# HongwenZhang/DaNet-DensePose2SMPL

Measured on NVIDIA H100. Metric: images/sec DaNet fwd bs=64 224x224 (HRNet-W48 + part regressors + SMPL LBS + IUV render), higher is better.
Workload: dtype split-f16 operands (hi+lo, 22 bits; 3 MMAs per K step), f32 accumulate

## Files before the change

### danet-densepose2smpl_b200/_lib.py

```python
import ctypes
import os

_HERE = os.path.dirname(os.path.abspath(__file__))
LIB_PATH = os.path.join(_HERE, "libdanet_b200.so")

c_int, c_i64, c_f, c_p = ctypes.c_int32, ctypes.c_int64, ctypes.c_float, ctypes.c_void_p


class SmplDesc(ctypes.Structure):
    _fields_ = [("num_verts", c_int), ("num_joints", c_int), ("num_betas", c_int),
                ("v_template", c_p), ("shapedirs", c_p), ("posedirs", c_p), ("J_regressor", c_p),
                ("lbs_weights", c_p), ("parents", c_p),
                ("num_selected", c_int), ("selected_verts", c_p),
                ("num_extra", c_int), ("J_regressor_extra", c_p),
                ("num_h36m", c_int), ("J_regressor_h36m", c_p),
                ("num_out_joints", c_int), ("joint_map", c_p)]


class RasterDesc(ctypes.Structure):
    _fields_ = [("num_smpl_verts", c_int), ("num_mesh_verts", c_int), ("vert_mapping", c_p),
                ("num_faces", c_int), ("faces", c_p), ("textures", c_p),
                ("orig_size", c_int), ("out_size", c_int), ("focal_length", c_f),
                ("near_plane", c_f), ("far_plane", c_f), ("tex_mode", c_int)]

# ... 30 lines not shown
SIGNATURES = {
    "danet_last_error": (ctypes.c_char_p, []),
    "danet_version": (c_int, []),
    "danet_device_info": (c_int, [c_p, c_p, c_p]),
    "danet_smpl_create": (c_int, [ctypes.POINTER(SmplDesc), ctypes.POINTER(c_p)]),
    "danet_smpl_destroy": (c_int, [c_p]),
    "danet_smpl_workspace_bytes": (c_i64, [c_p, c_int]),
    "danet_smpl_forward": (c_int, [c_p, c_int, c_p, c_p, c_int, c_p, c_p, c_p, c_p, c_p, c_p, c_int, c_p]),
    "danet_smpl_backward_workspace_bytes": (c_i64, [c_p, c_int]),
    "danet_smpl_backward": (c_int, [c_p, c_int, c_p, c_p, c_p, c_p, c_p, c_p, c_p, c_p]),
    "danet_rot6d_to_rotmat": (c_int, [c_int, c_p, c_p, c_p]),
    "danet_batch_rodrigues": (c_int, [c_int, c_p, c_p, c_int, c_p]),
    "danet_perspective_projection": (c_int, [c_int, c_int, c_p, c_p, c_p, c_p, c_p, c_p, c_p]),
    "danet_mpjpe_h36m": (c_int, [c_int, c_p, c_p, c_p, c_p]),
    "danet_body_uv_losses_workspace_bytes": (c_i64, [c_int, c_int]),
    "danet_body_uv_losses": (c_int, [c_int, c_int, c_int, c_int, c_i64, c_i64, c_p, c_p, c_p, c_p, c_p, c_p, c_p, c_p,
                                     c_p, c_f, c_f, c_p, c_p, c_p, c_p, c_p, c_p, c_p]),
    "danet_dp_uvia_losses_workspace_bytes": (c_i64, [c_int, c_int]),
    "danet_dp_uvia_losses": (c_int, [c_int, c_int, c_int, c_int] + [c_p] * 12 + [c_int, c_f, c_f, c_f] + [c_p] * 7),
    "danet_stn_kps_losses_workspace_bytes": (c_i64, [c_int, c_int]),
    "danet_stn_kps_losses": (c_int, [c_int, c_int, c_int, c_p, c_p, c_int, c_f, c_f, c_p, c_p, c_p, c_p, c_p]),
    "danet_part_iuv_targets": (c_int, [c_int, c_int, c_int, c_p, c_p, c_p, c_p, c_int, c_p, c_p]),
    "danet_raster_create": (c_int, [ctypes.POINTER(RasterDesc), ctypes.POINTER(c_p)]),
    "danet_raster_destroy": (c_int, [c_p]),
    "danet_raster_workspace_bytes": (c_i64, [c_p, c_int]),
    "danet_raster_iuv": (c_int, [c_p, c_int, c_p, c_p, c_p, c_p, c_p, c_p, c_p, c_p, c_p, c_p]),
    "danet_iuv_img2map": (c_int, [c_int, c_int, c_p, c_p, c_p, c_p, c_p, c_p]),
    "danet_conv_tc_packed_bytes": (c_i64, [ctypes.POINTER(ConvDesc)]),
    "danet_conv_tc_pack": (c_int, [ctypes.POINTER(ConvDesc), c_p, c_p, c_p]),
    "danet_conv_tc_supported": (c_int, [ctypes.POINTER(ConvDesc)]),
    "danet_conv_tc_geometry": (c_int, [ctypes.POINTER(ConvDesc), c_p]),
    "danet_conv_tc_cta_geometry": (c_int, [ctypes.POINTER(ConvDesc), c_p]),
    "danet_conv_tc_dispatch": (c_int, [ctypes.POINTER(ConvDesc), c_p]),
    "danet_conv_tc_group": (c_int, [c_int, ctypes.POINTER(ConvProblem), c_p]),
    "danet_conv_tc_config": (c_int, [c_int, ctypes.POINTER(ConvDesc), c_p]),
    "danet_conv_weights_simt": (c_int, [c_int] * 6 + [c_p, c_p, c_p]),
    "danet_conv_dgrad_pieces": (c_int, [c_int, c_int, c_p]),
    "danet_conv_dgrad_weights": (c_int, [c_int] * 5 + [c_p, c_int, c_int, c_p, c_p, c_p]),
    "danet_conv_dgrad_scatter": (c_int, [c_int] * 9 + [c_p, ctypes.POINTER(c_p), c_p, c_p, c_int, c_p, c_p]),
    "danet_conv_grad_split": (c_int, [c_int] * 4 + [c_p] * 5),
    "danet_conv_wgrad_workspace_bytes": (c_i64, [ctypes.POINTER(ConvDesc)]),
    "danet_conv_wgrad": (c_int, [ctypes.POINTER(ConvDesc), c_int, c_int, ctypes.POINTER(Act), ctypes.POINTER(Act), c_p, c_p,
                                 c_p, c_p, c_p]),
    "danet_conv_bias_grad_workspace_bytes": (c_i64, [c_int, c_int, c_int]),
    "danet_conv_bias_grad": (c_int, [c_int, c_int, c_int, c_p, c_p, c_p, c_p]),
    "danet_bn2d_workspace_bytes": (c_i64, [c_int, c_int, c_int]),
    "danet_bn2d_forward": (c_int, [c_int, c_int, c_int] + [c_p] * 5 + [c_int, c_f, c_f, c_p, c_int] + [c_p] * 5),
    "danet_bn2d_backward": (c_int, [c_int, c_int, c_int] + [c_p] * 5 + [c_int, c_int] + [c_p] * 6),
    "danet_maxpool3x3s2_nchw_forward": (c_int, [c_int] * 4 + [c_p] * 4),
    "danet_maxpool3x3s2_nchw_backward": (c_int, [c_int] * 4 + [c_p] * 4),
    "danet_global_avgpool_backward": (c_int, [c_int, c_int, c_p, c_p, c_p]),
    "danet_linear_backward": (c_int, [c_int] * 3 + [c_p] * 7),
    "danet_hr_fuse_forward": (c_int, [c_int] * 5 + [c_p, c_p, c_int, c_p, c_p]),
    "danet_hr_fuse_backward": (c_int, [c_int] * 5 + [c_p] * 4),
    "danet_part_crops_forward": (c_int, [c_int] * 3 + [c_p, c_p, c_int, c_p, c_p]),
    "danet_part_crops_backward": (c_int, [c_int] * 3 + [c_p, c_p, c_int, c_p, c_p]),
    "danet_part_thetas": (c_int, [c_int] * 3 + [c_p] * 4 + [c_f, c_p, c_f, c_p, c_f, c_int, c_p, c_p, c_p]),
    "danet_act_split": (c_int, [c_i64, c_p, c_p, c_p, c_p]),
    "danet_act_merge": (c_int, [c_i64, c_p, c_p, c_p, c_p]),
    "danet_global_avgpool": (c_int, [c_int, c_int, c_int, ctypes.POINTER(Act), c_p, c_p]),
    "danet_linear": (c_int, [c_int, c_int, c_int, c_p, c_p, c_p, c_p, c_p, c_p]),
    "danet_iuvmap_clean_nchw": (c_int, [c_int, c_int, c_int, c_int, c_p, c_p, c_p, c_p, c_p, c_p, c_p, c_p, c_p]),
    "danet_gcn_head_train_workspace_bytes": (c_i64, [c_int]),
    "danet_gcn_head_train_forward": (c_int, [c_int, ctypes.POINTER(GcnTrainParams), c_int] + [c_p] * 9),
    "danet_gcn_head_train_backward": (c_int, [c_int, ctypes.POINTER(GcnTrainParams), c_int] + [c_p] * 9),
    "danet_gcn_head_losses": (c_int, [c_int] + [c_p] * 6 + [c_f, c_f] + [c_p] * 5),
# ... 62 lines not shown
```

### danet-densepose2smpl_b200/csrc/conv_tc.cu

```cuda
#include "common.cuh"
#include "wgmma_f16.cuh"
#include "tc_ptx.cuh"
#include <cuda.h>
#include <cuda_fp16.h>
#include <mutex>
#include <utility>
#include <string.h>
#include <math.h>

namespace danet {
namespace tc {

constexpr int kTileH = 16, kTileW = 8;
constexpr int kConsFast = 2, kThreadsFast = (4 * kConsFast + 1) * 32;
constexpr int kWarpProd = 4 * kConsFast;
constexpr int kConsExact = 4, kThreadsExact = 4 * kConsExact * 32;
constexpr int kNtMaxExact = 64, kNtMaxFast = 256;
constexpr int kMaxAStages = 8, kMaxBStages = 8;
constexpr int kSmemMax = 227 * 1024;
constexpr int kSmemFixed = 2048;
constexpr int kSchedDepth = 4, kSchedAhead = 2, kSchedStatic = 3;
constexpr int kPackHeader = 1024;
constexpr int kSegMmas = 8;
__host__ __device__ constexpr bool seg_close(bool last_block, int seg_mmas) { return last_block || seg_mmas >= kSegMmas; }

struct alignas(64) Prob {
    CUtensorMap tm[2];
    const uint8_t* wpk; const float* bias;
    const float* res_f; const __half* res_hi; const __half* res_lo;
    float* y_f; __half* y_hi; __half* y_lo;
    int N, H, W, Cin, Cout, Ho, Wo, ks, stride, pad, relu, wsets, exact;
    int npa;
    int SWB, KCH, nchunks;
    int TG;
    int NT, ntn;
    int nstack, hs, box_h;
    int bpc;
    int par_py[4], par_px[4], ntap[4], ngrp[4], stage_bytes, sbo_a;
    int tapoff16[4][16];
    int tapidx[4][16];
    int tiles_w, tiles_h, tile_count;
    int rows_blk;
    int tap_bytes, b_block_bytes, nblk;
    long long blocks_per_set;
    unsigned long long m_ntn, m_tw, m_th, m_ws;
};

constexpr int kMaxProb = 6;
struct ArgsN {
    int nprob, total_units, na_stages, a_slot_bytes, nb_stages, b_slot_bytes;
    unsigned* sched;
    Prob p[kMaxProb];
    int unit_base[kMaxProb], unit_count[kMaxProb];
};

static unsigned long long magic40(int d) { return (1ull << 40) / (unsigned long long)d + 1ull; }

static bool make_prob(const danet_conv_desc* d, Prob* g) {
    if (!(d->stride == 1 || d->stride == 2) || !(d->ksize == 1 || d->ksize == 3 || d->ksize == 7) || d->pad != d->ksize / 2) return false;
    if (d->Cin % 8 != 0 || d->Cout % 8 != 0 || d->H < 1 || d->W < 1 || d->N < 1 || d->wsets < 1) return false;
    g->N = d->N; g->H = d->H; g->W = d->W; g->Cin = d->Cin; g->Cout = d->Cout; g->ks = d->ksize;
    g->pad = d->pad; g->stride = d->stride; g->relu = d->relu; g->wsets = d->wsets;
    g->exact = (d->flags & DANET_CONV_EXACT) ? 1 : 0;
    g->Ho = (d->H + 2 * d->pad - d->ksize) / d->stride + 1;
    g->Wo = (d->W + 2 * d->pad - d->ksize) / d->stride + 1;
    if (g->Ho < 1 || g->Wo < 1) return false;
    const int np = (d->Cout + 15) / 16 * 16;
    const int ntmax = g->exact ? kNtMaxExact : kNtMaxFast;
    g->ntn = (np + ntmax - 1) / ntmax;
    g->NT = ((np + g->ntn - 1) / g->ntn + 15) / 16 * 16;
    g->npa = 0;
    int max_ntap = 0, tr_max = 0, tc_max = 0;
    int tc_[4];
    for (int py = 0; py < d->stride; ++py)
        for (int px = 0; px < d->stride; ++px) {
            const int tr = py < d->ksize ? (d->ksize - 1 - py) / d->stride + 1 : 0;
            const int tcn = px < d->ksize ? (d->ksize - 1 - px) / d->stride + 1 : 0;
            if (tr * tcn == 0) continue;
            if (tr * tcn > 16) return false;
            const int a = g->npa++;
            g->par_py[a] = py; g->par_px[a] = px; g->ntap[a] = tr * tcn; tc_[a] = tcn;
            max_ntap = tr * tcn > max_ntap ? tr * tcn : max_ntap;
            tr_max = tr > tr_max ? tr : tr_max; tc_max = tcn > tc_max ? tcn : tc_max;
        }
    const int Hb = kTileH + tr_max - 1, Wb = kTileW + tc_max - 1;
    g->nstack = 1; g->hs = kTileH; g->box_h = Hb;
    if (d->stride == 1 && d->H + d->pad <= kTileH / 2) {
        g->hs = d->H + d->pad;
        g->box_h = d->H + 2 * d->pad;
    } else if (d->stride == 2 && g->Ho + tr_max - 1 <= kTileH / 2) {
        g->hs = g->box_h = g->Ho + tr_max - 1;
    }
    int swb = 128;
    const int c16 = (d->Cin + 15) / 16 * 16;
    while (swb > 32 && swb / 2 >= 2 * c16) swb /= 2;
    if (g->hs < kTileH && (g->hs * Wb * swb) % 128 != 0) { g->hs = kTileH; g->box_h = Hb; }
    if (g->hs < kTileH) g->nstack = kTileH / g->hs;
    g->SWB = swb; g->KCH = swb / 2;
    g->nchunks = (d->Cin + g->KCH - 1) / g->KCH;
    g->rows_blk = g->NT * (g->exact ? 2 : 1);
    g->tap_bytes = g->rows_blk * swb;
    int tg = max_ntap;
    while (tg > 1 && tg * g->tap_bytes > (g->exact ? 24 : 48) * 1024) --tg;
    g->TG = tg;
    g->b_block_bytes = (tg * g->tap_bytes + 1023) / 1024 * 1024;
    g->stage_bytes = Hb * Wb * swb; g->sbo_a = Wb * swb;
    g->bpc = 0;
    for (int a = 0; a < 4; ++a) {
        if (a >= g->npa) { g->par_py[a] = g->par_px[a] = g->ntap[a] = g->ngrp[a] = 0;
                           for (int k = 0; k < 16; ++k) g->tapoff16[a][k] = g->tapidx[a][k] = 0; continue; }
        g->ngrp[a] = (g->ntap[a] + tg - 1) / tg;
        g->bpc += g->ngrp[a];
        for (int k = 0; k < 16; ++k) { g->tapoff16[a][k] = 0; g->tapidx[a][k] = 0; }
        for (int k = 0; k < g->ntap[a]; ++k) {
            const int ti = k / tc_[a], tj = k % tc_[a];
            g->tapoff16[a][k] = ((ti * Wb + tj) * swb) >> 4;
            g->tapidx[a][k] = (g->par_py[a] + d->stride * ti) * d->ksize + (g->par_px[a] + d->stride * tj);
        }
    }
    g->nblk = g->nchunks * g->bpc;
    g->blocks_per_set = (long long)g->ntn * g->nblk;
    g->tiles_w = (g->Wo + kTileW - 1) / kTileW; g->tiles_h = (g->Ho + kTileH - 1) / kTileH;
    const long long groups = g->nstack == 1 ? d->N
                           : (long long)d->wsets * (((d->N + d->wsets - 1) / d->wsets + g->nstack - 1) / g->nstack);
    const long long tiles = groups * g->tiles_h * g->tiles_w * g->ntn;
    if (tiles >= (1 << 24) || g->wsets >= (1 << 16)) return false;
    if ((long long)d->N * g->Ho * g->Wo * d->Cout >= (1LL << 31) || (long long)d->N * d->H * d->W * d->Cin >= (1LL << 31)) return false;
    g->tile_count = (int)tiles;
    g->m_ntn = magic40(g->ntn); g->m_tw = magic40(g->tiles_w); g->m_th = magic40(g->tiles_h); g->m_ws = magic40(g->wsets);
    return true;
}

static int pair_count(const Prob& g) {
    const int U = g.tiles_h * g.tiles_w * g.ntn;
    const int groups = g.tile_count / U;
    if (g.tiles_h > 1) return groups * ((g.tiles_h + 1) / 2) * g.tiles_w * g.ntn;
    const int per_set = (groups + g.wsets - 1) / g.wsets;
    return (per_set + 1) / 2 * g.wsets * U;
}

static bool plan_rings(ArgsN* a) {
    int amax = 0, bmax = 0, need_a = 2, max_a = kMaxAStages;
    bool exact = false;
    for (int i = 0; i < a->nprob; ++i) {
        amax = a->p[i].stage_bytes > amax ? a->p[i].stage_bytes : amax;
        bmax = a->p[i].b_block_bytes > bmax ? a->p[i].b_block_bytes : bmax;
        if (a->p[i].exact) exact = true;
    }
    a->a_slot_bytes = (amax + 1023) / 1024 * 1024;
    a->b_slot_bytes = (bmax + 1023) / 1024 * 1024;
    if (exact) {
        a->a_slot_bytes *= 2;
        need_a = max_a = 3;
    }
    int nb = 3;
    int na = (kSmemMax - kSmemFixed - nb * a->b_slot_bytes) / a->a_slot_bytes;
    if (na < need_a) { nb = 2; na = (kSmemMax - kSmemFixed - nb * a->b_slot_bytes) / a->a_slot_bytes; }
    if (na < need_a) return false;
    if (na > max_a) na = max_a;
    while (nb < kMaxBStages && kSmemFixed + na * a->a_slot_bytes + (nb + 1) * a->b_slot_bytes <= kSmemMax) ++nb;
    a->na_stages = na; a->nb_stages = nb;
    return true;
}

__device__ __forceinline__ uint64_t make_desc(uint32_t saddr, uint32_t sbo_bytes, uint32_t swb) {
    const uint32_t mode = swb == 128 ? 1u : (swb == 64 ? 2u : 3u);
    const uint32_t lo = ((saddr >> 4) & 0x3FFFu) | (1u << 16);
    const uint32_t hi = ((sbo_bytes >> 4) & 0x3FFFu) | (mode << 30);
    return ((uint64_t)hi << 32) | lo;
}
__host__ __device__ __forceinline__ uint32_t swz(uint32_t off, uint32_t mask) { return off ^ (((off >> 7) & mask) << 4); }
__host__ __device__ __forceinline__ int mdiv(int x, unsigned long long m) { return (int)(((unsigned long long)(unsigned)x * m) >> 40); }

struct TileCoord { int nt, tw, th, img0, ws; };
__host__ __device__ __forceinline__ void group_coord(const Prob& g, int grp, TileCoord& c) {
    const int bg = mdiv(grp, g.m_ws);
    c.ws = grp - bg * g.wsets;
    c.img0 = c.ws + g.wsets * bg * g.nstack;
}
__device__ __forceinline__ TileCoord decode_tile(const Prob& g, int t) {
    TileCoord c;
    int r = mdiv(t, g.m_ntn); c.nt = t - r * g.ntn;
    int r2 = mdiv(r, g.m_tw); c.tw = r - r2 * g.tiles_w;
    const int grp = mdiv(r2, g.m_th); c.th = r2 - grp * g.tiles_h;
    group_coord(g, grp, c);
    return c;
}

__host__ __device__ __forceinline__ TileCoord pair_coord(const Prob& g, int pp, int h) {
    TileCoord c;
    const int r = mdiv(pp, g.m_ntn); c.nt = pp - r * g.ntn;
    const int outer = mdiv(r, g.m_tw); c.tw = r - outer * g.tiles_w;
    int grp;
    if (g.tiles_h > 1) {
        const int th2 = (g.tiles_h + 1) >> 1;
        grp = outer / th2;
        c.th = 2 * (outer - grp * th2) + h;
    } else {
        const int q = mdiv(outer, g.m_ws);
        grp = (2 * q + h) * g.wsets + (outer - q * g.wsets);
        c.th = 0;
    }
    group_coord(g, grp, c);
    return c;
}

struct Ring { int as, bs; uint32_t aph, bph; };

struct Smem { uint32_t sA, sB, bar_a_full, bar_a_empty, bar_b_full, bar_b_empty; };

constexpr uint32_t kOffSchedFull = 512, kOffSchedEmpty = kOffSchedFull + 8 * kSchedDepth;
constexpr uint32_t kOffSchedRing = kOffSchedFull + 16 * kSchedDepth, kOffCursor = 640, kOffPark = 768;

enum CursorField {
    kCurSeq, kCurPub, kCurPubEnd,
    kCurPi,
    kCurC, kCurSlot, kCurStep,
    kCurH0, kCurH1, kCurW0,
    kCurImg0, kCurImg1, kCurBlk,
    kCurFa, kCurFb,
    kCurRa, kCurRb,
    kCurAs, kCurBs, kCurAph, kCurBph,
    kCurFields
};
static_assert(kOffCursor + 4 * kCurFields <= kOffPark && kOffPark + 4 * 32 <= 1024, "barrier region layout");

__device__ __forceinline__ int sched_next(const Smem& S, int seq) {
// ... 19 lines not shown
    asm volatile("ld.shared.s32 %0, [%1];" : "=r"(v) : "r"(cur + 4 * f) : "memory");
    return v;
}
__device__ __forceinline__ void cur_set(uint32_t cur, int f, int v) {
    asm volatile("st.shared.s32 [%0], %1;" ::"r"(cur + 4 * f), "r"(v) : "memory");
}

__device__ __forceinline__ void produce(const ArgsN& a, const Smem& S, int dA, int dB) {
    const uint32_t cur = S.bar_a_full + kOffCursor;
    cur_set(cur, kCurRa, cur_get(cur, kCurRa) + dA);
    cur_set(cur, kCurRb, cur_get(cur, kCurRb) + dB);
#pragma unroll 1
    for (;;) {
        if (cur_get(cur, kCurPi) < 0) {
#pragma unroll 1
            while (cur_get(cur, kCurPub) <= cur_get(cur, kCurSeq) + kSchedAhead && !cur_get(cur, kCurPubEnd)) {
                const int pub = cur_get(cur, kCurPub), rs = pub & (kSchedDepth - 1);
                mbar_wait_inl(S.bar_a_full + kOffSchedEmpty + 8 * rs, ((pub / kSchedDepth) & 1) ^ 1);
                const int t = sched_unit(a, pub, [&] { return __shfl_sync(0xffffffffu, atom_inc_elect(a.sched), 0); });
                if (t == a.total_units) cur_set(cur, kCurPubEnd, 1);
                st_arrive_elect(S.bar_a_full + kOffSchedRing + 4 * rs, t, S.bar_a_full + kOffSchedFull + 8 * rs);
                cur_set(cur, kCurPub, pub + 1);
            }
            int pair;
            asm volatile("ld.shared.s32 %0, [%1];" : "=r"(pair)
                         : "r"(S.bar_a_full + kOffSchedRing + 4 * (cur_get(cur, kCurSeq) & (kSchedDepth - 1))) : "memory");
            pair = __shfl_sync(0xffffffffu, pair, 0);
            if (pair >= a.total_units) return;
            const int pi = unit_prob(a, pair);
            const Prob& P = a.p[pi];
            const int pp = pair - a.unit_base[pi];
            {
                const TileCoord tc = pair_coord(P, pp, 0);
                cur_set(cur, kCurH0, tc.th * kTileH * P.stride - P.pad);
                cur_set(cur, kCurW0, tc.tw * kTileW * P.stride - P.pad);
                cur_set(cur, kCurImg0, tc.img0);
                cur_set(cur, kCurBlk, tc.ws * (int)P.blocks_per_set + tc.nt * P.nblk);
            }
            {
                const TileCoord tc = pair_coord(P, pp, 1);
                cur_set(cur, kCurH1, tc.th * kTileH * P.stride - P.pad);
                cur_set(cur, kCurImg1, tc.img0);
            }
            cur_set(cur, kCurC, 0); cur_set(cur, kCurSlot, 0); cur_set(cur, kCurStep, 0);
            cur_set(cur, kCurPi, pi);
        }
        const Prob& P = a.p[cur_get(cur, kCurPi)];
        const int step = cur_get(cur, kCurStep);
        if (step < 2) {
            if (cur_get(cur, kCurFa) >= cur_get(cur, kCurRa) + a.na_stages) return;
            {
                const int as = cur_get(cur, kCurAs);
                mbar_wait_inl(S.bar_a_empty + 8 * as, ((cur_get(cur, kCurAph) >> as) & 1) ^ 1);
                mbar_expect_tx_elect(S.bar_a_full + 8 * as, 2u * P.nstack * P.box_h * P.sbo_a);
            }
#pragma unroll 1
            for (int k = 0; k < 2 * P.nstack; ++k) {
                const int h = k >= P.nstack ? 1 : 0, n = k - h * P.nstack, slot = cur_get(cur, kCurSlot), as = cur_get(cur, kCurAs);
                tma_load_4d_elect(S.sA + as * a.a_slot_bytes + h * (a.a_slot_bytes >> 1) + n * P.hs * P.sbo_a,
                                  &P.tm[step], cur_get(cur, kCurC) * P.KCH, cur_get(cur, kCurW0) + P.par_px[slot],
                                  cur_get(cur, kCurH0 + h) + P.par_py[slot], cur_get(cur, kCurImg0 + h) + n * P.wsets,
                                  S.bar_a_full + 8 * as);
            }
            const int as = cur_get(cur, kCurAs);
            cur_set(cur, kCurAph, cur_get(cur, kCurAph) ^ (1 << as));
            cur_set(cur, kCurAs, as + 1 == a.na_stages ? 0 : as + 1);
            cur_set(cur, kCurFa, cur_get(cur, kCurFa) + 1);
            cur_set(cur, kCurStep, step + 1);
        } else {
            if (cur_get(cur, kCurFb) >= cur_get(cur, kCurRb) + a.nb_stages) return;
            {
                const int bs = cur_get(cur, kCurBs);
                mbar_wait_inl(S.bar_b_empty + 8 * bs, ((cur_get(cur, kCurBph) >> bs) & 1) ^ 1);
                const uint32_t bar = S.bar_b_full + 8 * bs;
                mbar_expect_tx_elect(bar, (uint32_t)P.b_block_bytes);
                bulk_g2s_elect(S.sB + bs * a.b_slot_bytes, P.wpk + kPackHeader + (long long)cur_get(cur, kCurBlk) * P.b_block_bytes,
                               (uint32_t)P.b_block_bytes, bar);
                cur_set(cur, kCurBph, cur_get(cur, kCurBph) ^ (1 << bs));
                cur_set(cur, kCurBs, bs + 1 == a.nb_stages ? 0 : bs + 1);
            }
            cur_set(cur, kCurFb, cur_get(cur, kCurFb) + 1);
            cur_set(cur, kCurBlk, cur_get(cur, kCurBlk) + 1);
            const int slot = cur_get(cur, kCurSlot);
            if (step - 1 < P.ngrp[slot]) cur_set(cur, kCurStep, step + 1);
            else {
                cur_set(cur, kCurStep, 0);
                if (slot + 1 < P.npa) cur_set(cur, kCurSlot, slot + 1);
                else {
                    cur_set(cur, kCurSlot, 0);
                    if (cur_get(cur, kCurC) + 1 < P.nchunks) cur_set(cur, kCurC, cur_get(cur, kCurC) + 1);
                    else { cur_set(cur, kCurPi, -1); cur_set(cur, kCurSeq, cur_get(cur, kCurSeq) + 1); }
                }
            }
        }
    }
}


__device__ __forceinline__ int ring_take(uint32_t bar_full, int& idx, uint32_t& ph, int n) {
    const int s = idx;
    mbar_wait_inl(bar_full + 8 * s, (ph >> s) & 1u);
    ph ^= 1u << s; if (++idx == n) idx = 0;
    return s;
}

struct TileOut { uint32_t eoff[2]; bool ok[2]; int cw, boff; };
template <int NT>
__device__ __forceinline__ TileOut tile_out(const Prob& P, const TileCoord& tc, int wg, int w4, int lane) {
    TileOut o;
    const int prow0 = 8 * wg + 2 * w4, pcol = lane >> 2, cq = 2 * (lane & 3);
    const int Cout = P.Cout, Wo = P.Wo, Ho = P.Ho;
    const int ow = tc.tw * kTileW + pcol;
#pragma unroll
    for (int r = 0; r < 2; ++r) {
        const int prow = prow0 + r;
        int oh = tc.th * kTileH + prow, img = tc.img0;
        bool row_ok = oh < Ho;
        if (P.nstack > 1) {
            const int n = prow / P.hs;
            oh = prow - n * P.hs; img = tc.img0 + n * P.wsets;
            row_ok = oh < Ho && n < P.nstack && img < P.N;
        }
        o.ok[r] = row_ok && ow < Wo;
        o.eoff[r] = ((uint32_t)(img * Ho + oh) * Wo + ow) * Cout + tc.nt * NT + cq;
    }
    o.cw = Cout - tc.nt * NT;
    o.boff = tc.ws * Cout + tc.nt * NT + cq;
    return o;
}

template <int W, class Off>
__device__ __forceinline__ uint32_t mma_taps(float* d0, float* d1, uint64_t ad, uint64_t bd, const Prob& P, int slot, int k0,
                                             int ntk, int kv, Off tap16, uint32_t acc) {
#pragma unroll 1
    for (int tt = 0; tt < ntk; ++tt) {
        const uint32_t toff = (uint32_t)P.tapoff16[slot][k0 + tt];
#pragma unroll
        for (int kk = 0; kk < 4; ++kk) {
            if (kk >= kv) break;
            Wgmma<W>::mma(d0, d1, ad + toff + 2 * kk, bd + tt * tap16 + 2 * kk, acc);
            acc = 1;
        }
    }
    return acc;
}

template <int NT, class Value>
__device__ __forceinline__ void store_out(const Prob& P, const TileOut& o, float inv_scale, Value value) {
    const int relu = P.relu;
    float* __restrict__ y_f = P.y_f; __half* __restrict__ y_hi = P.y_hi; __half* __restrict__ y_lo = P.y_lo;
#pragma unroll
// ... 278 lines not shown
            default: __trap();
        }
#undef DANET_NT_CASE
    }
    sched_rearm(a);
}

__global__ void __launch_bounds__(kThreadsFast, 1)
k_conv_tc_fast(const __grid_constant__ ArgsN a) {
    const Smem S = carve_smem(a);
    const int warp = warp_index(), lane = threadIdx.x & 31;
    start_cta(a, S, kConsFast, kWarpProd, 1, warp, lane);
    if (warp == kWarpProd) {
        if (lane == 0) {
            int as = 0, bs = 0; uint32_t aph = 0, bph = 0;
            int pub = 0; bool ended = false;
            for (int seq = 0;; ++seq) {
                while (pub <= seq + kSchedAhead && !ended) {
                    const int slot = pub & (kSchedDepth - 1);
                    mbar_wait(S.bar_a_full + kOffSchedEmpty + 8 * slot, ((pub / kSchedDepth) & 1) ^ 1);
                    const int t = sched_unit(a, pub, [&] { return (int)atomicAdd(a.sched, 1u); });
                    ended = t == a.total_units;
                    asm volatile("st.shared.s32 [%0], %1;" ::"r"(S.bar_a_full + kOffSchedRing + 4 * slot), "r"(t) : "memory");
                    mbar_arrive(S.bar_a_full + kOffSchedFull + 8 * slot);
                    ++pub;
                }
                int tile;
                asm volatile("ld.shared.s32 %0, [%1];" : "=r"(tile) : "r"(S.bar_a_full + kOffSchedRing + 4 * (seq & (kSchedDepth - 1))) : "memory");
                if (tile >= a.total_units) break;
                if (seq == 0) pdl_wait();
                const int pi = unit_prob(a, tile);
                const Prob& P = a.p[pi];
                const TileCoord tc = decode_tile(P, tile - a.unit_base[pi]);
                const int h0 = tc.th * kTileH * P.stride - P.pad, w0 = tc.tw * kTileW * P.stride - P.pad;
                const uint8_t* src = P.wpk + kPackHeader + ((long long)tc.ws * P.blocks_per_set + (long long)tc.nt * P.nblk) * P.b_block_bytes;
                int b = 0;
                for (int c = 0; c < P.nchunks; ++c)
                    for (int slot = 0; slot < P.npa; ++slot) {
                        mbar_wait(S.bar_a_empty + 8 * as, ((aph >> as) & 1u) ^ 1u);
                        if (P.nstack > 1) {
                            const uint32_t box_bytes = (uint32_t)(P.box_h * P.sbo_a);
                            mbar_expect_tx(S.bar_a_full + 8 * as, box_bytes * P.nstack);
                            for (int n = 0; n < P.nstack; ++n)
                                tma_load_4d(S.sA + as * a.a_slot_bytes + n * P.hs * P.sbo_a, &P.tm[0], c * P.KCH,
                                            w0 + P.par_px[slot], h0 + P.par_py[slot], tc.img0 + n * P.wsets, S.bar_a_full + 8 * as);
                        } else {
                            mbar_expect_tx(S.bar_a_full + 8 * as, (uint32_t)P.stage_bytes);
                            tma_load_4d(S.sA + as * a.a_slot_bytes, &P.tm[0], c * P.KCH, w0 + P.par_px[slot], h0 + P.par_py[slot],
                                        tc.img0, S.bar_a_full + 8 * as);
                        }
                        aph ^= 1u << as;
                        if (++as == a.na_stages) as = 0;
                        for (int t = 0; t < P.ngrp[slot]; ++t, ++b) {
                            mbar_wait(S.bar_b_empty + 8 * bs, ((bph >> bs) & 1u) ^ 1u);
                            mbar_expect_tx(S.bar_b_full + 8 * bs, (uint32_t)P.b_block_bytes);
                            bulk_g2s(S.sB + bs * a.b_slot_bytes, src + (long long)b * P.b_block_bytes, (uint32_t)P.b_block_bytes,
                                     S.bar_b_full + 8 * bs);
                            bph ^= 1u << bs;
                            if (++bs == a.nb_stages) bs = 0;
                        }
                    }
            }
        }
    } else {
        const int wg = warp >> 2, w4 = warp & 3;
        const bool leader = (threadIdx.x & 127) == 0;
        Ring R = {0, 0, 0u, 0u};
        float accs[kNtMaxFast / 2];
        pdl_wait();
        for (int seq = 0;; ++seq) {
            int tile = 0;
            if (lane == 0) tile = sched_next(S, seq);
            tile = __shfl_sync(0xffffffffu, tile, 0);
            if (tile >= a.total_units) break;
            const int pi = unit_prob(a, tile);
// ... 119 lines not shown
    using namespace tc;
    ArgsN a;
    {
        const danet_conv_desc* dp[kMaxProb];
        DANET_CHECK(n >= 1 && n <= kMaxProb, "danet_conv_tc_group: 1..%d problems per launch (got %d)", kMaxProb, n);
        for (int i = 0; i < n; ++i) dp[i] = &probs[i].d;
        if (configure_group(n, dp, &a) != 0) return -1;
    }
    int order[kMaxProb];
    double tcost[kMaxProb];
    for (int i = 0; i < n; ++i) {
        const Prob& P = a.p[i];
        int taps = 0;
        for (int s2 = 0; s2 < P.npa; ++s2) taps += P.ntap[s2];
        tcost[i] = (double)taps * ((P.Cin + 15) / 16) * (P.exact ? 2.0 : 1.0) * (128 + P.NT * (P.exact ? 1.5 : 1.0));
        order[i] = i;
    }
    for (int i = 1; i < n; ++i)
        for (int j = i; j > 0 && tcost[j] > tcost[j - 1]; --j) {
            std::swap(a.p[j], a.p[j - 1]); std::swap(tcost[j], tcost[j - 1]); std::swap(order[j], order[j - 1]);
        }
    int tiles = 0;
    for (int i = 0; i < n; ++i) {
        Prob& P = a.p[i];
        const danet_conv_problem& q = probs[order[i]];
        DANET_CHECK(q.x.hi && q.w_packed && (q.y.hi || q.y.f32), "danet_conv_tc_group: problem %d: null x.hi / weights / output", order[i]);
        DANET_CHECK(!P.exact || q.x.lo, "danet_conv_tc_group: problem %d: exact mode needs the x.lo plane", order[i]);
        P.wpk = (const uint8_t*)q.w_packed; P.bias = q.bias;
        P.res_f = q.res.f32; P.res_hi = (const __half*)q.res.hi; P.res_lo = (const __half*)q.res.lo;
        if (P.res_f) { P.res_hi = nullptr; P.res_lo = nullptr; }
        P.y_f = q.y.f32; P.y_hi = (__half*)q.y.hi; P.y_lo = (__half*)q.y.lo;
        const CUtensorMapSwizzle sw = P.SWB == 128 ? CU_TENSOR_MAP_SWIZZLE_128B : (P.SWB == 64 ? CU_TENSOR_MAP_SWIZZLE_64B : CU_TENSOR_MAP_SWIZZLE_32B);
        for (int h = 0; h < (P.exact ? 2 : 1); ++h)
            if (encode_nhwc_f16(&P.tm[h], h ? q.x.lo : q.x.hi, P.N, P.H, P.W, P.Cin, P.KCH, P.sbo_a / P.SWB, P.box_h, sw, P.stride) != 0) return -1;
        if (!P.exact) P.tm[1] = P.tm[0];
        tiles += P.tile_count;
        DANET_CHECK(tiles < (1 << 24), "danet_conv_tc_group: too many tiles");
        a.unit_base[i] = a.total_units;
        a.unit_count[i] = P.exact ? pair_count(P) : P.tile_count;
        a.total_units += a.unit_count[i];
    }
    int dev = 0;
    DANET_CUDA(cudaGetDevice(&dev));
    DANET_CHECK(dev >= 0 && dev < 64, "conv_tc: device ordinal %d out of range", dev);
    {
        std::lock_guard<std::mutex> lk(g_tc_mu);
        if (first_use_on_current_device(&g_tc_devs) != 0) {
            DANET_CUDA(cudaDeviceGetAttribute(&g_sm_count[dev], cudaDevAttrMultiProcessorCount, dev));
            DANET_CUDA(cudaFuncSetAttribute(k_conv_tc_fast, cudaFuncAttributeMaxDynamicSharedMemorySize, kSmemMax));
            DANET_CUDA(cudaFuncSetAttribute(k_conv_tc_exact, cudaFuncAttributeMaxDynamicSharedMemorySize, kSmemMax));
            DANET_CUDA(cudaMalloc((void**)&g_sched[dev], kSchedSlots * 2 * sizeof(unsigned)));
            DANET_CUDA(cudaMemset(g_sched[dev], 0, kSchedSlots * 2 * sizeof(unsigned)));
        }
        a.sched = g_sched[dev] + 2 * (g_sched_seq[dev]++ % kSchedSlots);
    }
    const int smem_bytes = kSmemFixed + a.na_stages * a.a_slot_bytes + a.nb_stages * a.b_slot_bytes;
    const int cap = g_sm_count[dev];
    const int grid = a.total_units < cap ? a.total_units : cap;
    cudaLaunchConfig_t cfg = {};
    cfg.gridDim = dim3(grid); cfg.blockDim = dim3(a.p[0].exact ? kThreadsExact : kThreadsFast);
    cfg.dynamicSmemBytes = smem_bytes;
    cfg.stream = stream;
    cudaLaunchAttribute at[1];
    at[0].id = cudaLaunchAttributeProgrammaticStreamSerialization;
    at[0].val.programmaticStreamSerializationAllowed = 1;
    cfg.attrs = at; cfg.numAttrs = 1;
    if (a.p[0].exact) { DANET_CUDA(cudaLaunchKernelEx(&cfg, k_conv_tc_exact, a)); }
// ... 2 lines not shown
    return 0;
}

}

using namespace danet;

extern "C" int danet_conv_tc_supported(const danet_conv_desc* d) {
    tc::Prob g;
    if (!d || !tc::make_prob(d, &g)) return 0;
    tc::ArgsN* a = new tc::ArgsN();
    a->nprob = 1; a->p[0] = g;
    const bool ok = tc::plan_rings(a);
    delete a;
    return ok ? 1 : 0;
}

extern "C" int64_t danet_conv_tc_packed_bytes(const danet_conv_desc* d) {
    tc::Prob g;
    if (!d || !tc::make_prob(d, &g)) return 0;
    return tc::kPackHeader + (int64_t)d->wsets * g.blocks_per_set * g.b_block_bytes;
}

extern "C" int danet_conv_tc_geometry(const danet_conv_desc* d, int64_t* out) {
    tc::Prob g;
    if (!d || !out || !tc::make_prob(d, &g)) return -1;
    int64_t ksteps = 0, taps = 0, a_bytes = 0;
    for (int c = 0; c < g.nchunks; ++c) {
        const int kreal = (g.Cin - c * g.KCH + 15) / 16;
        ksteps += kreal < g.KCH / 16 ? kreal : g.KCH / 16;
    }
    for (int s = 0; s < g.npa; ++s) {
        taps += g.ntap[s];
        a_bytes += g.nstack > 1 ? (int64_t)g.nstack * g.box_h * g.sbo_a : g.stage_bytes;
    }
    out[0] = tc::kTileH; out[1] = tc::kTileW; out[2] = g.tile_count; out[3] = g.nstack;
    out[4] = g.exact ? 3 : 1;
    out[5] = (int64_t)tc::kTileH * tc::kTileW * g.NT * 16 * ksteps * taps;
    out[6] = a_bytes * g.nchunks * (g.exact ? 2 : 1);
    out[7] = (int64_t)g.nblk * g.b_block_bytes;
    return 0;
}

extern "C" int danet_conv_tc_cta_geometry(const danet_conv_desc* d, int64_t* out) {
    int64_t t[8];
    if (danet_conv_tc_geometry(d, t) != 0) return -1;
    tc::Prob g;
    tc::make_prob(d, &g);
    const int tiles = g.exact ? 2 : 1;
    out[0] = tiles;
    out[1] = g.exact ? tc::pair_count(g) : g.tile_count;
    out[2] = t[7];
    out[3] = t[6] * tiles;
    return 0;
}

extern "C" int danet_conv_tc_dispatch(const danet_conv_desc* d, int64_t* out) {
    tc::Prob g;
    if (!d || !out || !tc::make_prob(d, &g)) return -1;
    const int kmma = g.KCH / 16;
    int kv_last = 0, max_ntap = 0, max_ngrp = 0;
    int64_t closes = 0, longest = 0, at_plane_end = 0, mid_plane = 0;
    int seg = 0;
    for (int c = 0; c < g.nchunks; ++c) {
        const int kreal = (g.Cin - c * g.KCH + 15) >> 4;
        const int kv = kreal < kmma ? kreal : kmma;
        kv_last = kv;
        for (int slot = 0; slot < g.npa; ++slot) {
            max_ntap = g.ntap[slot] > max_ntap ? g.ntap[slot] : max_ntap;
            max_ngrp = g.ngrp[slot] > max_ngrp ? g.ngrp[slot] : max_ngrp;
            for (int tg = 0; tg < g.ngrp[slot]; ++tg) {
                const int ntk = g.TG < g.ntap[slot] - tg * g.TG ? g.TG : g.ntap[slot] - tg * g.TG;
                const bool plane_end = tg == g.ngrp[slot] - 1;
                const bool last = c == g.nchunks - 1 && slot == g.npa - 1 && plane_end;
                seg += ntk * kv;
                if (!g.exact || !tc::seg_close(last, seg)) continue;
                ++closes;
                longest = seg > longest ? seg : longest;
                if (!last) ++(plane_end ? at_plane_end : mid_plane);
                seg = 0;
            }
        }
    }
    int64_t pairs = 0, past = 0;
    if (g.exact) {
        pairs = tc::pair_count(g);
        const int inner = g.tiles_w * g.ntn;
        for (int64_t o = 0; o < pairs / inner; ++o) {
            const tc::TileCoord t = tc::pair_coord(g, (int)(o * inner), 1);
            if (g.tiles_h > 1 ? t.th >= g.tiles_h : t.img0 >= g.N) past += inner;
        }
    }
    const int64_t r[DANET_CONV_DISPATCH_FIELDS] = {
        g.NT, g.ntn, g.Cout - (g.ntn - 1) * g.NT, g.SWB, g.KCH, g.nchunks, kv_last, g.npa, max_ntap, g.TG, max_ngrp,
        g.nstack, g.hs, g.tiles_h, g.tiles_w, g.nblk, closes, longest, at_plane_end, mid_plane,
        g.exact ? (g.tiles_h > 1 ? 1 : 2) : 0, pairs, past};
    for (int i = 0; i < DANET_CONV_DISPATCH_FIELDS; ++i) out[i] = r[i];
    return 0;
}

extern "C" int danet_conv_tc_pack(const danet_conv_desc* d, const float* w_simt, void* w_packed, danet_stream_t stream) {
    tc::Prob g;
    DANET_CHECK(d && tc::make_prob(d, &g), "danet_conv_tc_pack: shape not supported by the tensor-core path");
    DANET_CHECK(w_simt && w_packed, "danet_conv_tc_pack: null pointer");
    cudaStream_t st = (cudaStream_t)stream;
    const long long nw = (long long)d->wsets * d->ksize * d->ksize * d->Cin * d->Cout;
    const int rc = pow2_scale(w_simt, nw, (float*)w_packed, tc::kPackHeader / 4, st);
    if (rc != 0) return rc;
    const long long total = (long long)g.wsets * g.blocks_per_set * (g.b_block_bytes / 2);
    tc::k_pack<<<(unsigned)((total + 255) / 256), 256, 0, st>>>(g, w_simt, (__half*)((uint8_t*)w_packed + tc::kPackHeader),
                                                                 (const float*)w_packed);
    DANET_LAUNCH_CHECK();
    return 0;
}

extern "C" int danet_conv_tc_config(int32_t n, const danet_conv_desc* descs, int32_t* stages) {
    DANET_CHECK(descs && stages, "danet_conv_tc_config: null pointer");
    const danet_conv_desc* dp[tc::kMaxProb];
    DANET_CHECK(n >= 1 && n <= tc::kMaxProb, "danet_conv_tc_config: 1..%d problems (got %d)", tc::kMaxProb, n);
    for (int i = 0; i < n; ++i) dp[i] = &descs[i];
    tc::ArgsN* a = new tc::ArgsN();
    const int rc = configure_group(n, dp, a);
    if (rc == 0) { stages[0] = a->na_stages; stages[1] = a->nb_stages; }
    delete a;
    return rc;
}

extern "C" int danet_conv_tc_group(int32_t n, const danet_conv_problem* probs, danet_stream_t stream) {
    DANET_CHECK(probs, "danet_conv_tc_group: null problem list");
    for (int i = 0; i < n; ++i) if (probs[i].d.N == 0) { DANET_CHECK(n == 1, "danet_conv_tc_group: empty problem in a group"); return 0; }
// ... 19 lines not shown
```

### include/danet_b200.h

```cpp
#ifndef DANET_B200_H
#define DANET_B200_H
#include <stdint.h>
#ifdef __cplusplus
extern "C" {
#endif

typedef void* danet_stream_t;
typedef struct danet_smpl*   danet_smpl_t;
typedef struct danet_raster* danet_raster_t;

const char* danet_last_error(void);
int danet_version(void);
int danet_device_info(int* sm_count, int* cc_major, int* cc_minor);

typedef struct {
    int32_t num_verts;
    int32_t num_joints;
    int32_t num_betas;
    const float* v_template;
    const float* shapedirs;
    const float* posedirs;
    const float* J_regressor;
    const float* lbs_weights;
    const int32_t* parents;
// ... 57 lines not shown
                           const float* theta, int32_t align_corners, float* out, danet_stream_t stream);

typedef struct {
    int32_t num_smpl_verts;
    int32_t num_mesh_verts;
    const int32_t* vert_mapping;
    int32_t num_faces;
    const int32_t* faces;
    const float* textures;
    int32_t orig_size;
    int32_t out_size;
    float focal_length;
    float near_plane, far_plane;
    int32_t tex_mode;
} danet_raster_desc;

int danet_raster_create(const danet_raster_desc* desc, danet_raster_t* out);
int danet_raster_destroy(danet_raster_t h);
int64_t danet_raster_workspace_bytes(danet_raster_t h, int32_t B);
int danet_raster_iuv(danet_raster_t h, int32_t B, const float* verts, const float* cam, float* img,
                     int32_t* face_idx, float* maps_u, float* maps_v, float* maps_i, float* maps_ann,
                     void* workspace, danet_stream_t stream);
int danet_iuv_img2map(int32_t B, int32_t S, const float* img, float* maps_u, float* maps_v,
                      float* maps_i, float* maps_ann, danet_stream_t stream);

typedef struct {
    int32_t N, H, W, Cin;
    int32_t Cout, ksize, stride, pad;
    int32_t wsets;
    int32_t relu;
    int32_t flags;
} danet_conv_desc;
#define DANET_CONV_EXACT 4

typedef struct { float* f32; void* hi; void* lo; } danet_act;

typedef struct {
    danet_conv_desc d;
    danet_act x, res, y;
    const void* w_packed;
    const float* bias;
} danet_conv_problem;
int danet_conv_tc_group(int32_t n, const danet_conv_problem* problems, danet_stream_t stream);
int danet_conv_tc_config(int32_t n, const danet_conv_desc* descs, int32_t* stages);
int64_t danet_conv_tc_packed_bytes(const danet_conv_desc* d);
int danet_conv_tc_pack(const danet_conv_desc* d, const float* w_simt, void* w_packed, danet_stream_t stream);
int danet_conv_tc_supported(const danet_conv_desc* d);
int danet_conv_tc_geometry(const danet_conv_desc* d, int64_t* out);
int danet_conv_tc_cta_geometry(const danet_conv_desc* d, int64_t* out);
#define DANET_CONV_DISPATCH_FIELDS 23
int danet_conv_tc_dispatch(const danet_conv_desc* d, int64_t* out);
int danet_act_split(int64_t n, const float* x, void* hi, void* lo, danet_stream_t stream);
int danet_act_merge(int64_t n, const void* hi, const void* lo, float* y, danet_stream_t stream);

int danet_conv_weights_simt(int32_t wsets, int32_t cout, int32_t cin, int32_t ksize, int32_t Cout, int32_t Cin,
                            const float* w, float* w_simt, danet_stream_t stream);
typedef struct { int32_t a, b, K, tr, tc, jr0, jr1, jc0, jc1; } danet_dgrad_piece;
int32_t danet_conv_dgrad_pieces(int32_t ksize, int32_t stride, danet_dgrad_piece* pieces);
int danet_conv_dgrad_weights(int32_t wsets, int32_t cout, int32_t cin, int32_t ksize, int32_t stride,
                             const danet_dgrad_piece* piece, int32_t Cout, int32_t Cin, const float* w, float* w_out,
                             danet_stream_t stream);
int danet_conv_dgrad_scatter(int32_t N, int32_t C, int32_t H, int32_t W, int32_t Cp, int32_t stride, int32_t Hc, int32_t Wc,
                             int32_t npieces, const danet_dgrad_piece* pieces, const float* const* maps,
                             const float* scale, const float* bias, int32_t groups, float* y, danet_stream_t stream);
int danet_conv_grad_split(int32_t N, int32_t C, int32_t HW, int32_t Cp, const float* dy, void* hi, void* lo, float* scale,
                          danet_stream_t stream);
int64_t danet_conv_wgrad_workspace_bytes(const danet_conv_desc* d);
int danet_conv_wgrad(const danet_conv_desc* d, int32_t cout, int32_t cin, const danet_act* x, const danet_act* dy,
                     const float* dy_scale, const float* x_scale, float* dW, void* workspace, danet_stream_t stream);
int64_t danet_conv_bias_grad_workspace_bytes(int32_t N, int32_t C, int32_t HW);
int danet_conv_bias_grad(int32_t N, int32_t C, int32_t HW, const float* dy, float* db, void* workspace, danet_stream_t stream);

int64_t danet_bn2d_workspace_bytes(int32_t N, int32_t C, int32_t HW);
int danet_bn2d_forward(int32_t N, int32_t C, int32_t HW, const float* x, const float* weight, const float* bias,
                       const float* running_mean, const float* running_var, int32_t training, float momentum, float eps,
                       const float* residual, int32_t relu, float* y, double* save, float* new_running, void* workspace,
                       danet_stream_t stream);
int danet_bn2d_backward(int32_t N, int32_t C, int32_t HW, const float* x, const float* y, const float* dy,
                        const float* weight, const double* save, int32_t training, int32_t relu, float* dx, float* dweight,
                        float* dbias, float* dresidual, void* workspace, danet_stream_t stream);
int danet_maxpool3x3s2_nchw_forward(int32_t N, int32_t C, int32_t H, int32_t W, const float* x, float* y, uint8_t* slot,
                                    danet_stream_t stream);
int danet_maxpool3x3s2_nchw_backward(int32_t N, int32_t C, int32_t H, int32_t W, const float* dy, const uint8_t* slot,
                                     float* dx, danet_stream_t stream);
// ... 66 lines not shown
```

Before: 1616.

## Add full-width row-band tile mapping for implicit-GEMM convolutions

Adds an alternative output tiling where each 128-pixel tile covers a band of full output rows instead of a fixed 16x8 patch. The TMA box, smem stage layout, tile decode, pair scheduling and epilogue coordinate math are adapted for this band mode. It is chosen automatically when it gives fewer tile pairs without a larger stage. The aim is to cut padding waste and redundant halo loads on layers whose widths are not multiples of 8. It adds a mapping query API and an opt-out flag. The risk is mis-indexing in the new path, since the producer still uses kTileW for the column offset.

```diff
diff --git a/danet-densepose2smpl_b200/_lib.py b/danet-densepose2smpl_b200/_lib.py
--- a/danet-densepose2smpl_b200/_lib.py
+++ b/danet-densepose2smpl_b200/_lib.py
@@ -86,6 +86,7 @@
     "danet_conv_tc_geometry": (c_int, [ctypes.POINTER(ConvDesc), c_p]),
     "danet_conv_tc_cta_geometry": (c_int, [ctypes.POINTER(ConvDesc), c_p]),
     "danet_conv_tc_dispatch": (c_int, [ctypes.POINTER(ConvDesc), c_p]),
+    "danet_conv_tc_mapping": (c_int, [ctypes.POINTER(ConvDesc), c_p]),
     "danet_conv_tc_group": (c_int, [c_int, ctypes.POINTER(ConvProblem), c_p]),
     "danet_conv_tc_config": (c_int, [c_int, ctypes.POINTER(ConvDesc), c_p]),
     "danet_conv_weights_simt": (c_int, [c_int] * 6 + [c_p, c_p, c_p]),
diff --git a/danet-densepose2smpl_b200/csrc/conv_tc.cu b/danet-densepose2smpl_b200/csrc/conv_tc.cu
--- a/danet-densepose2smpl_b200/csrc/conv_tc.cu
+++ b/danet-densepose2smpl_b200/csrc/conv_tc.cu
@@ -35,6 +35,8 @@
     int TG;
     int NT, ntn;
     int nstack, hs, box_h;
+    int rb, tile_rows, tile_cols;
+    int box_w, box_bytes;
     int bpc;
     int par_py[4], par_px[4], ntap[4], ngrp[4], stage_bytes, sbo_a;
     int tapoff16[4][16];
@@ -56,7 +58,7 @@
 
 static unsigned long long magic40(int d) { return (1ull << 40) / (unsigned long long)d + 1ull; }
 
-static bool make_prob(const danet_conv_desc* d, Prob* g) {
+static bool make_prob_as(const danet_conv_desc* d, Prob* g, bool bands) {
     if (!(d->stride == 1 || d->stride == 2) || !(d->ksize == 1 || d->ksize == 3 || d->ksize == 7) || d->pad != d->ksize / 2) return false;
     if (d->Cin % 8 != 0 || d->Cout % 8 != 0 || d->H < 1 || d->W < 1 || d->N < 1 || d->wsets < 1) return false;
     g->N = d->N; g->H = d->H; g->W = d->W; g->Cin = d->Cin; g->Cout = d->Cout; g->ks = d->ksize;
@@ -83,7 +85,7 @@
             max_ntap = tr * tcn > max_ntap ? tr * tcn : max_ntap;
             tr_max = tr > tr_max ? tr : tr_max; tc_max = tcn > tc_max ? tcn : tc_max;
         }
-    const int Hb = kTileH + tr_max - 1, Wb = kTileW + tc_max - 1;
+    int Hb = kTileH + tr_max - 1, Wb = kTileW + tc_max - 1;
     g->nstack = 1; g->hs = kTileH; g->box_h = Hb;
     if (d->stride == 1 && d->H + d->pad <= kTileH / 2) {
         g->hs = d->H + d->pad;
@@ -96,6 +98,14 @@
     while (swb > 32 && swb / 2 >= 2 * c16) swb /= 2;
     if (g->hs < kTileH && (g->hs * Wb * swb) % 128 != 0) { g->hs = kTileH; g->box_h = Hb; }
     if (g->hs < kTileH) g->nstack = kTileH / g->hs;
+    g->rb = 0; g->tile_rows = kTileH; g->tile_cols = kTileW;
+    if (bands) {
+        Wb = g->Wo + tc_max - 1;
+        if (g->nstack > 1 || Wb > kTileH * kTileW) return false;
+        g->rb = 1; g->tile_rows = kTileH * kTileW / Wb; g->tile_cols = Wb;
+        Hb = g->box_h = g->tile_rows + tr_max - 1;
+        g->hs = g->tile_rows;
+    }
     g->SWB = swb; g->KCH = swb / 2;
     g->nchunks = (d->Cin + g->KCH - 1) / g->KCH;
     g->rows_blk = g->NT * (g->exact ? 2 : 1);
@@ -104,7 +114,8 @@
     while (tg > 1 && tg * g->tap_bytes > (g->exact ? 24 : 48) * 1024) --tg;
     g->TG = tg;
     g->b_block_bytes = (tg * g->tap_bytes + 1023) / 1024 * 1024;
-    g->stage_bytes = Hb * Wb * swb; g->sbo_a = Wb * swb;
+    g->stage_bytes = Hb * Wb * swb; g->sbo_a = (g->rb ? 8 : Wb) * swb;
+    g->box_w = Wb; g->box_bytes = g->box_h * Wb * swb;
     g->bpc = 0;
     for (int a = 0; a < 4; ++a) {
         if (a >= g->npa) { g->par_py[a] = g->par_px[a] = g->ntap[a] = g->ngrp[a] = 0;
@@ -120,7 +131,8 @@
     }
     g->nblk = g->nchunks * g->bpc;
     g->blocks_per_set = (long long)g->ntn * g->nblk;
-    g->tiles_w = (g->Wo + kTileW - 1) / kTileW; g->tiles_h = (g->Ho + kTileH - 1) / kTileH;
+    g->tiles_w = (g->Wo + g->tile_cols - 1) / g->tile_cols;
+    g->tiles_h = (g->Ho + g->tile_rows - 1) / g->tile_rows;
     const long long groups = g->nstack == 1 ? d->N
                            : (long long)d->wsets * (((d->N + d->wsets - 1) / d->wsets + g->nstack - 1) / g->nstack);
     const long long tiles = groups * g->tiles_h * g->tiles_w * g->ntn;
@@ -134,8 +146,9 @@
 static int pair_count(const Prob& g) {
     const int U = g.tiles_h * g.tiles_w * g.ntn;
     const int groups = g.tile_count / U;
+    const int per_set = (groups + g.wsets - 1) / g.wsets;
+    if (g.rb) return (per_set * g.tiles_h + 1) / 2 * g.wsets * g.ntn;
     if (g.tiles_h > 1) return groups * ((g.tiles_h + 1) / 2) * g.tiles_w * g.ntn;
-    const int per_set = (groups + g.wsets - 1) / g.wsets;
     return (per_set + 1) / 2 * g.wsets * U;
 }
 
@@ -163,6 +176,16 @@
     return true;
 }
 
+static bool make_prob(const danet_conv_desc* d, Prob* g) {
+    if (!make_prob_as(d, g, false)) return false;
+    if ((d->flags & DANET_CONV_NO_ROWBANDS) || g->nstack > 1 || g->Ho <= kTileH || g->Wo <= 2 * kTileW) return true;
+    Prob b;
+    if (!make_prob_as(d, &b, true) || pair_count(b) >= pair_count(*g)) return true;
+    if ((b.stage_bytes + 1023) / 1024 > (g->stage_bytes + 1023) / 1024) return true;
+    *g = b;
+    return true;
+}
+
 __device__ __forceinline__ uint64_t make_desc(uint32_t saddr, uint32_t sbo_bytes, uint32_t swb) {
     const uint32_t mode = swb == 128 ? 1u : (swb == 64 ? 2u : 3u);
     const uint32_t lo = ((saddr >> 4) & 0x3FFFu) | (1u << 16);
@@ -192,7 +215,11 @@
     const int r = mdiv(pp, g.m_ntn); c.nt = pp - r * g.ntn;
     const int outer = mdiv(r, g.m_tw); c.tw = r - outer * g.tiles_w;
     int grp;
-    if (g.tiles_h > 1) {
+    if (g.rb) {
+        const int q = mdiv(outer, g.m_ws), L = 2 * q + h, i = mdiv(L, g.m_th);
+        grp = i * g.wsets + (outer - q * g.wsets);
+        c.th = L - i * g.tiles_h;
+    } else if (g.tiles_h > 1) {
         const int th2 = (g.tiles_h + 1) >> 1;
         grp = outer / th2;
         c.th = 2 * (outer - grp * th2) + h;
@@ -278,14 +305,14 @@
             const int pp = pair - a.unit_base[pi];
             {
                 const TileCoord tc = pair_coord(P, pp, 0);
-                cur_set(cur, kCurH0, tc.th * kTileH * P.stride - P.pad);
+                cur_set(cur, kCurH0, tc.th * P.tile_rows * P.stride - P.pad);
                 cur_set(cur, kCurW0, tc.tw * kTileW * P.stride - P.pad);
                 cur_set(cur, kCurImg0, tc.img0);
                 cur_set(cur, kCurBlk, tc.ws * (int)P.blocks_per_set + tc.nt * P.nblk);
             }
             {
                 const TileCoord tc = pair_coord(P, pp, 1);
-                cur_set(cur, kCurH1, tc.th * kTileH * P.stride - P.pad);
+                cur_set(cur, kCurH1, tc.th * P.tile_rows * P.stride - P.pad);
                 cur_set(cur, kCurImg1, tc.img0);
             }
             cur_set(cur, kCurC, 0); cur_set(cur, kCurSlot, 0); cur_set(cur, kCurStep, 0);
@@ -298,7 +325,7 @@
             {
                 const int as = cur_get(cur, kCurAs);
                 mbar_wait_inl(S.bar_a_empty + 8 * as, ((cur_get(cur, kCurAph) >> as) & 1) ^ 1);
-                mbar_expect_tx_elect(S.bar_a_full + 8 * as, 2u * P.nstack * P.box_h * P.sbo_a);
+                mbar_expect_tx_elect(S.bar_a_full + 8 * as, 2u * P.nstack * P.box_bytes);
             }
 #pragma unroll 1
             for (int k = 0; k < 2 * P.nstack; ++k) {
@@ -356,13 +383,16 @@
     TileOut o;
     const int prow0 = 8 * wg + 2 * w4, pcol = lane >> 2, cq = 2 * (lane & 3);
     const int Cout = P.Cout, Wo = P.Wo, Ho = P.Ho;
-    const int ow = tc.tw * kTileW + pcol;
 #pragma unroll
     for (int r = 0; r < 2; ++r) {
         const int prow = prow0 + r;
-        int oh = tc.th * kTileH + prow, img = tc.img0;
+        int oh = tc.th * kTileH + prow, ow = tc.tw * kTileW + pcol, img = tc.img0;
         bool row_ok = oh < Ho;
-        if (P.nstack > 1) {
+        if (P.rb) {
+            const int pos = 8 * prow + pcol, rr = pos / P.tile_cols;
+            oh = tc.th * P.tile_rows + rr; ow = pos - rr * P.tile_cols;
+            row_ok = rr < P.tile_rows && oh < Ho;
+        } else if (P.nstack > 1) {
             const int n = prow / P.hs;
             oh = prow - n * P.hs; img = tc.img0 + n * P.wsets;
             row_ok = oh < Ho && n < P.nstack && img < P.N;
@@ -707,15 +737,14 @@
                 const int pi = unit_prob(a, tile);
                 const Prob& P = a.p[pi];
                 const TileCoord tc = decode_tile(P, tile - a.unit_base[pi]);
-                const int h0 = tc.th * kTileH * P.stride - P.pad, w0 = tc.tw * kTileW * P.stride - P.pad;
+                const int h0 = tc.th * P.tile_rows * P.stride - P.pad, w0 = tc.tw * kTileW * P.stride - P.pad;
                 const uint8_t* src = P.wpk + kPackHeader + ((long long)tc.ws * P.blocks_per_set + (long long)tc.nt * P.nblk) * P.b_block_bytes;
                 int b = 0;
                 for (int c = 0; c < P.nchunks; ++c)
                     for (int slot = 0; slot < P.npa; ++slot) {
                         mbar_wait(S.bar_a_empty + 8 * as, ((aph >> as) & 1u) ^ 1u);
                         if (P.nstack > 1) {
-                            const uint32_t box_bytes = (uint32_t)(P.box_h * P.sbo_a);
-                            mbar_expect_tx(S.bar_a_full + 8 * as, box_bytes * P.nstack);
+                            mbar_expect_tx(S.bar_a_full + 8 * as, (uint32_t)P.box_bytes * P.nstack);
                             for (int n = 0; n < P.nstack; ++n)
                                 tma_load_4d(S.sA + as * a.a_slot_bytes + n * P.hs * P.sbo_a, &P.tm[0], c * P.KCH,
                                             w0 + P.par_px[slot], h0 + P.par_py[slot], tc.img0 + n * P.wsets, S.bar_a_full + 8 * as);
@@ -901,7 +930,7 @@
         P.y_f = q.y.f32; P.y_hi = (__half*)q.y.hi; P.y_lo = (__half*)q.y.lo;
         const CUtensorMapSwizzle sw = P.SWB == 128 ? CU_TENSOR_MAP_SWIZZLE_128B : (P.SWB == 64 ? CU_TENSOR_MAP_SWIZZLE_64B : CU_TENSOR_MAP_SWIZZLE_32B);
         for (int h = 0; h < (P.exact ? 2 : 1); ++h)
-            if (encode_nhwc_f16(&P.tm[h], h ? q.x.lo : q.x.hi, P.N, P.H, P.W, P.Cin, P.KCH, P.sbo_a / P.SWB, P.box_h, sw, P.stride) != 0) return -1;
+            if (encode_nhwc_f16(&P.tm[h], h ? q.x.lo : q.x.hi, P.N, P.H, P.W, P.Cin, P.KCH, P.box_w, P.box_h, sw, P.stride) != 0) return -1;
         if (!P.exact) P.tm[1] = P.tm[0];
         tiles += P.tile_count;
         DANET_CHECK(tiles < (1 << 24), "danet_conv_tc_group: too many tiles");
@@ -970,9 +999,9 @@
     }
     for (int s = 0; s < g.npa; ++s) {
         taps += g.ntap[s];
-        a_bytes += g.nstack > 1 ? (int64_t)g.nstack * g.box_h * g.sbo_a : g.stage_bytes;
-    }
-    out[0] = tc::kTileH; out[1] = tc::kTileW; out[2] = g.tile_count; out[3] = g.nstack;
+        a_bytes += (int64_t)g.nstack * g.box_bytes;
+    }
+    out[0] = g.tile_rows; out[1] = g.tile_cols; out[2] = g.tile_count; out[3] = g.nstack;
     out[4] = g.exact ? 3 : 1;
     out[5] = (int64_t)tc::kTileH * tc::kTileW * g.NT * 16 * ksteps * taps;
     out[6] = a_bytes * g.nchunks * (g.exact ? 2 : 1);
@@ -1026,14 +1055,22 @@
         const int inner = g.tiles_w * g.ntn;
         for (int64_t o = 0; o < pairs / inner; ++o) {
             const tc::TileCoord t = tc::pair_coord(g, (int)(o * inner), 1);
-            if (g.tiles_h > 1 ? t.th >= g.tiles_h : t.img0 >= g.N) past += inner;
+            if (g.tiles_h > 1 && !g.rb ? t.th >= g.tiles_h : t.img0 >= g.N) past += inner;
         }
     }
     const int64_t r[DANET_CONV_DISPATCH_FIELDS] = {
         g.NT, g.ntn, g.Cout - (g.ntn - 1) * g.NT, g.SWB, g.KCH, g.nchunks, kv_last, g.npa, max_ntap, g.TG, max_ngrp,
         g.nstack, g.hs, g.tiles_h, g.tiles_w, g.nblk, closes, longest, at_plane_end, mid_plane,
-        g.exact ? (g.tiles_h > 1 ? 1 : 2) : 0, pairs, past};
+        g.exact ? (g.rb ? 3 : (g.tiles_h > 1 ? 1 : 2)) : 0, pairs, past};
     for (int i = 0; i < DANET_CONV_DISPATCH_FIELDS; ++i) out[i] = r[i];
+    return 0;
+}
+
+extern "C" int danet_conv_tc_mapping(const danet_conv_desc* d, int64_t* out) {
+    tc::Prob g;
+    if (!d || !out || !tc::make_prob(d, &g)) return -1;
+    const int64_t r[DANET_CONV_MAPPING_FIELDS] = {g.rb, g.tile_rows, g.tile_cols, g.box_h, g.box_w, g.stage_bytes};
+    for (int i = 0; i < DANET_CONV_MAPPING_FIELDS; ++i) out[i] = r[i];
     return 0;
 }
 
diff --git a/include/danet_b200.h b/include/danet_b200.h
--- a/include/danet_b200.h
+++ b/include/danet_b200.h
@@ -113,6 +113,7 @@
     int32_t flags;
 } danet_conv_desc;
 #define DANET_CONV_EXACT 4
+#define DANET_CONV_NO_ROWBANDS 8
 
 typedef struct { float* f32; void* hi; void* lo; } danet_act;
 
@@ -131,6 +132,8 @@
 int danet_conv_tc_cta_geometry(const danet_conv_desc* d, int64_t* out);
 #define DANET_CONV_DISPATCH_FIELDS 23
 int danet_conv_tc_dispatch(const danet_conv_desc* d, int64_t* out);
+#define DANET_CONV_MAPPING_FIELDS 6
+int danet_conv_tc_mapping(const danet_conv_desc* d, int64_t* out);
 int danet_act_split(int64_t n, const float* x, void* hi, void* lo, danet_stream_t stream);
 int danet_act_merge(int64_t n, const void* hi, const void* lo, float* y, danet_stream_t stream);
 
```

Measured after the change: 1628, median of 6. No clear change (+0.7%).
